# eigenkernel/eigenkernel

Hardware: AMD Instinct MI355X
Metric: eigenpairs/s (full spectrum) + achieved fp64 TFLOP/s vs roofline, N=16384 GEP (higher is better)
Workload: dtype f64

## Files before the change

### eigenkernel_amd/csrc/ek_api_internal.h

```cpp
#pragma once
#include "../../include/ek_hip.h"
#include "../../include/ek_hip_debug.h"
#include "ek_common.h"

#include <rccl/rccl.h>

#include <chrono>
#include <cstdlib>
#include <cstring>
#include <mutex>
#include <vector>

namespace ek {
namespace batched {
struct Desc {
  double *A, *B, *w, *Z;
  int n, lda, ldb, ldz, index, pad;
};
static_assert(sizeof(Desc) == 56, "the table's entry");
}

namespace api {

struct Context {
// ... 60 lines not shown
struct GridCell { int nb, nprow, npcol, myrow, mycol; };

extern ek_hip_allgatherv_fn g_allgatherv;
extern void *g_allgatherv_user;

int pad_ld(int n);
int h2d_matrix(int m, int n, const double *h, int ldh, double *d, int ldd, hipStream_t s);
int d2h_matrix(int m, int n, const double *d, int ldd, double *h, int ldh, hipStream_t s);
int fetch_info(int *info);
void poison_foreign_strips(hipStream_t s, int n, double *A, int lda, int P, int rank);
void count_mismatch(hipStream_t s, int m, int n, const double *X, int ldx, const double *Y, int ldy, int lower,
                    unsigned long long *count);

struct Comm {
  bool on = false;
  bool host = false;
  ncclComm_t comm = nullptr;
  int nranks = 0, rank = 0;
  int err = 0;
};
extern Comm g_comm;
constexpr int kPotrfRlMin = 1024;
extern int g_two_stage_min;
int two_stage_min();
int dist_min_ranks();
void comm_teardown();
SytrdExchange team_exchange(int nteam, int n = 0);
void team_sendrecv(hipStream_t s, int npeers, const int *peers, double *const *send, const size_t *send_counts,
                   double *const *recv, const size_t *recv_counts);
int comm_any(int local);
int comm_agree(int local_rc);
const char *comm_error_string();

void gather_band_strips(hipStream_t s, int n, int nmem, int rank0, double *const *ABs, const SytrdExchange &x);

}
}
```

### eigenkernel_amd/csrc/ek_comm.hip

```cpp
#include "ek_api_internal.h"
#include <dlfcn.h>

namespace ek {
namespace api {

struct Rccl {
  void *h = nullptr;
  ncclResult_t (*GetUniqueId)(ncclUniqueId *) = nullptr;
  ncclResult_t (*CommInitRank)(ncclComm_t *, int, ncclUniqueId, int) = nullptr;
  ncclResult_t (*CommDestroy)(ncclComm_t) = nullptr;
  ncclResult_t (*AllReduce)(const void *, void *, size_t, ncclDataType_t, ncclRedOp_t, ncclComm_t, hipStream_t) = nullptr;
  const char *(*GetErrorString)(ncclResult_t) = nullptr;
  ncclResult_t (*Broadcast)(const void *, void *, size_t, ncclDataType_t, int, ncclComm_t, hipStream_t) = nullptr;
  ncclResult_t (*GroupStart)() = nullptr;
  ncclResult_t (*GroupEnd)() = nullptr;
  ncclResult_t (*AllGather)(const void *, void *, size_t, ncclDataType_t, ncclComm_t, hipStream_t) = nullptr;
  ncclResult_t (*Send)(const void *, size_t, ncclDataType_t, int, ncclComm_t, hipStream_t) = nullptr;
  ncclResult_t (*Recv)(void *, size_t, ncclDataType_t, int, ncclComm_t, hipStream_t) = nullptr;
  int load() {
    if (h) return 0;
    const char *names[] = {getenv("EK_HIP_RCCL_LIB"), "librccl.so.1", "librccl.so", "/opt/rocm/lib/librccl.so.1"};
    for (const char *nm : names) {
      if (!nm || !*nm) continue;
      h = dlopen(nm, RTLD_NOW | RTLD_GLOBAL);
// ... 29 lines not shown
}

void rccl_allgatherv(hipStream_t s, int nmem, int, double *const *bufs, const size_t *offs,
                     const size_t *counts, int nranks, void *) {
  if (nmem != 1 || !g_comm.on || nranks != g_comm.nranks) { if (!g_comm.err) g_comm.err = (int)ncclInvalidUsage; return; }
  bool side_by_side = g_rccl.AllGather != nullptr && counts[0] > 0;
  for (int q = 1; q < nranks && side_by_side; ++q) side_by_side = counts[q] == counts[0] && offs[q] == offs[0] + (size_t)q * counts[0];
  if (side_by_side) {
    const ncclResult_t ra = g_rccl.AllGather(bufs[0] + offs[g_comm.rank], bufs[0] + offs[0], counts[0], ncclDouble, g_comm.comm, s);
    if (ra != ncclSuccess && !g_comm.err) g_comm.err = (int)ra;
    return;
  }
  ncclResult_t r = g_rccl.GroupStart();
  for (int root = 0; root < nranks && r == ncclSuccess; ++root)
    if (counts[root] > 0)
      r = g_rccl.Broadcast(bufs[0] + offs[root], bufs[0] + offs[root], counts[root], ncclDouble, root, g_comm.comm, s);
  const ncclResult_t r2 = g_rccl.GroupEnd();
  if (r == ncclSuccess) r = r2;
  if (r != ncclSuccess && !g_comm.err) g_comm.err = (int)r;
}


int g_two_stage_min = -1;
int two_stage_min() {
  if (g_two_stage_min >= 0) return g_two_stage_min;
  static int env = -2;
  if (env == -2) { const char *e = getenv("EK_HIP_TWO_STAGE_MIN"); env = e ? atoi(e) : -1; }
  return env >= 0 ? env : 512;
}

int dist_min_ranks() {
  const char *e = getenv("EK_HIP_DIST_MIN_RANKS");
  return e ? atoi(e) : 3;
}

std::vector<double> g_hx_send, g_hx_recv;
void host_allreduce(hipStream_t s, int nmem, double *const *bufs, size_t count, void *) {
  if (nmem != 1 || !g_comm.on || !g_allgatherv) { if (!g_comm.err) g_comm.err = (int)ncclInvalidUsage; return; }
  const int P = g_comm.nranks;
  g_hx_send.resize(count); g_hx_recv.resize(count * P);
  std::vector<long long> counts(P, (long long)count), displs(P);
  for (int r = 0; r < P; ++r) displs[r] = (long long)r * (long long)count;
  bool ok = hipStreamSynchronize(s) == hipSuccess &&
            hipMemcpy(g_hx_send.data(), bufs[0], count * 8, hipMemcpyDeviceToHost) == hipSuccess;
  if (ok) ok = g_allgatherv(g_hx_send.data(), (long long)count, g_hx_recv.data(), counts.data(), displs.data(),
                            g_allgatherv_user) == 0;
// ... 222 lines not shown
```

### eigenkernel_amd/csrc/ek_common.h

```cpp
#pragma once
#include <hip/hip_runtime.h>
#include <cstddef>
#include <cstdint>
#include <cstdio>

#define EK_HIP_CHECK(expr)                                                              \
  do {                                                                                  \
    hipError_t _e = (expr);                                                             \
    if (_e != hipSuccess) {                                                             \
      fprintf(stderr, "[ek_hip] %s failed at %s:%d: %s\n", #expr, __FILE__, __LINE__,   \
              hipGetErrorString(_e));                                                   \
      return -1000 - (int)_e;                                                           \
    }                                                                                   \
  } while (0)

namespace ek {

constexpr int kWave = 64;

inline int ceil_div(int a, int b) { return (a + b - 1) / b; }
inline int round_up(int a, int b) { return ceil_div(a, b) * b; }

struct GemmDesc {
  int M, N, K;
// ... 138 lines not shown
void symv_profile_collect(double *seconds, long long *launches, double *bytes);

constexpr int kBandW = 64;
size_t sy2sb_work_bytes(int n);
void sy2sb_lower(hipStream_t s, hipStream_t s2, int n, double *A, int lda, double *Vall, int ldv, double *tau1,
                 int *d_flag, void *work);

struct Sy2sbMember { double *A; int lda; double *Vall; int ldv; double *tau1; int *d_flag; void *work; int rank; };
size_t sy2sb_dist_work_bytes(int n, int nranks);
void sy2sb_lower_dist(hipStream_t s, hipStream_t s2, int n, int nmem, const Sy2sbMember *mem, const SytrdExchange &x);
void sy2sb_dist_set_lookahead(int min_rows);
void sy2sb_dist_profile(bool on);
void sy2sb_dist_profile_collect(double *seconds, int P);

size_t sb2st_work_bytes(int n, bool with_records = true);
size_t sb2st_record_bytes(int n);
constexpr int kBandLd = 2 * kBandW;
double *sb2st_band(void *work, int n);
void pack_band(hipStream_t s, int n, const double *A, int lda, double *AB );
void sb2st_lower(hipStream_t s, int n, const double *A, int lda, double *d, double *e, double *V2, int ldv2,
                 int *d_flag, void *work, bool band_packed = false, int chase_mode = 0);
void sb2st_apply_q2(hipStream_t s, int n, int ncols, const double *V2, int ldv2, double *Z, int ldz, int *d_flag,
                    void *work, double *records = nullptr);

size_t stedc_work_bytes(int n, int nsel = -1);
bool stedc_compact(int n, int nsel);
struct StedcSelect { int nsel, nb, npcol, mycol; int first = 0; };
struct StedcTeam { int nranks; int rank; const SytrdExchange *x; int levels; };
int stedc_team_levels(int n, int nranks);
void stedc_team_set_levels(int levels);
void stedc_team_profile(bool on);
void stedc_team_profile_collect(double *seconds);
void stedc(hipStream_t s, int n, const double *d, const double *e, double *w, double *Z,
           int ldz, void *work, int *d_info, const StedcSelect *sel = nullptr, double *d_flops = nullptr,
           double *wscratch = nullptr, const StedcTeam *team = nullptr);

size_t stebz_work_bytes(int n);
void stebz(hipStream_t s, int n, const double *d, const double *e, int il, int iu, double *w, void *work);
int stebz_set_lanes(int lanes);
int *stebz_window(hipStream_t s, int n, const double *d, const double *e, double vl, double vu, void *work);

size_t ormtr_work_bytes(int n, int ncols, int ncols_global = -1);
void ormtr_lower(hipStream_t s, int n, int ncols, const double *V, int ldv, const double *tau,
                 double *Z, int ldz, void *work, int ncols_global = -1);
size_t ormtr_prep_bytes(int n);
void ormtr_prepare(hipStream_t s, int n, const double *V, int ldv, const double *tau, void *prep);
// ... 18 lines not shown
```

### eigenkernel_amd/csrc/ek_debug.hip

```cpp
#include "ek_api_internal.h"

using namespace ek;
using namespace ek::api;

extern "C" {

int ek_hip_potrf_team(int n, double *B_loc, const int desc_B[9], int nteam, long long *mismatch) {
  if (n < 0) return -1;
  if (!B_loc && n > 0) return -2;
  int rc = check_desc(desc_B, 3, n, n); if (rc) return rc;
  if (nteam < 0 || nteam > kMaxTeam) return -4;
  rc = ensure_init(); if (rc) return rc;
  if (mismatch) *mismatch = 0;
  if (n == 0) return 0;
  std::lock_guard<std::mutex> lk(g_mu);
  if (nteam == 0 && !g_comm.on) return -4;
  hipStream_t s = g_ctx.stream;
  const int ld = pad_ld(n), nblk = ceil_div(n, kDiagNB);
  const int nmem = nteam > 0 ? nteam : 1, P = nteam > 0 ? nteam : g_comm.nranks;
  const size_t wb = potrf_dist_work_bytes(n, ld, P);
  const size_t per = al((size_t)ld * ld * 8) + al((size_t)nblk * kDiagNB * kDiagNB * 8) + al(wb) + 256;
  void *ws;
  rc = workspace(per * nmem + 256, &ws);
  if (rc) return rc;
// ... 289 lines not shown
  double *dd = a.get<double>(ld), *de = a.get<double>(ld);
  EK_HIP_CHECK(hipMemsetAsync(dA, 0, (size_t)ld * ld * 8, s));
  EK_HIP_CHECK(hipMemsetAsync(dV2, 0, (size_t)ld * ld * 8, s));
  EK_HIP_CHECK(hipMemsetAsync(dd, 0, 2 * al((size_t)ld * 8), s));
  EK_HIP_CHECK(hipMemsetAsync(g_ctx.d_info, 0, 4 * sizeof(int), s));
  rc = h2d_matrix(n, n, A, lda, dA, ld, s); if (rc) return rc;
  sb2st_lower(s, n, dA, ld, dd, de, dV2, ld, g_ctx.d_info + 2, work);
  if (ncols > 0) {
    rc = h2d_matrix(n, ncols, Z, ldz, dZ, ld, s); if (rc) return rc;
    sb2st_apply_q2(s, n, ncols, dV2, ld, dZ, ld, g_ctx.d_info + 2, work);
    rc = d2h_matrix(n, ncols, dZ, ld, Z, ldz, s); if (rc) return rc;
  }
  EK_HIP_CHECK(hipGetLastError());
  EK_HIP_CHECK(hipMemcpyAsync(d, dd, (size_t)n * 8, hipMemcpyDeviceToHost, s));
  if (n > 1) EK_HIP_CHECK(hipMemcpyAsync(e, de, (size_t)(n - 1) * 8, hipMemcpyDeviceToHost, s));
  int f = 0;
  EK_HIP_CHECK(hipMemcpyAsync(&f, g_ctx.d_info + 2, sizeof(int), hipMemcpyDeviceToHost, s));
  EK_HIP_CHECK(hipStreamSynchronize(s));
  if (flag) *flag = f;
  return 0;
}

int ek_hip_debug_set_two_stage(int min_order) { g_two_stage_min = min_order; return 0; }

int ek_hip_profile_kernels(int enable) {
  int rc = ensure_init(); if (rc) return rc;
  std::lock_guard<std::mutex> lk(g_mu);
  EK_HIP_CHECK(hipStreamSynchronize(g_ctx.stream));
  kprof_enable(enable != 0);
  return 0;
}
int ek_hip_profile_kernels_get(double *seconds, long long *launches) {
  int rc = ensure_init(); if (rc) return rc;
  std::lock_guard<std::mutex> lk(g_mu);
  EK_HIP_CHECK(hipStreamSynchronize(g_ctx.stream));
  kprof_collect(seconds, launches);
  return 0;
}

int ek_hip_debug_last_solve_stats(double *out, int count) {
  std::lock_guard<std::mutex> lk(g_mu);
  for (int i = 0; i < count && i < 8; ++i) out[i] = g_ctx.stats[i];
  return 0;
}

int ek_hip_debug_two_stage_timing(int n, int ncols, int reps, double *seconds, int *flag) {
// ... 407 lines not shown
```

### eigenkernel_amd/csrc/ek_sb2st.hip

```cpp
#include "ek_common.h"

#include <cstdlib>
#include <type_traits>
#include <vector>

namespace ek {
namespace {

typedef double double4_t __attribute__((ext_vector_type(4)));

constexpr int SB = kBandW;
constexpr int LDAB = 2 * SB;
constexpr int DLD = SB + 1;

__device__ __forceinline__ double ld_sc1(const double *p) {
  return __longlong_as_double((long long)__hip_atomic_load((const unsigned long long *)p, __ATOMIC_RELAXED,
                                                           __HIP_MEMORY_SCOPE_AGENT));
}
__device__ __forceinline__ void st_sc1(double *p, double v) {
  __hip_atomic_store((unsigned long long *)p, (unsigned long long)__double_as_longlong(v), __ATOMIC_RELAXED,
                     __HIP_MEMORY_SCOPE_AGENT);
}
template <int CTRL>
__device__ __forceinline__ double dpp_mov(double v) {
// ... 1095 lines not shown
    if (nw == 16) hipLaunchKernelGGL(chase_kernel<16>, dim3(nwg), dim3(1024), 0, s, c);
    else if (nw == 8) hipLaunchKernelGGL(chase_kernel<8>, dim3(nwg), dim3(512), 0, s, c);
    else hipLaunchKernelGGL(chase_kernel<4>, dim3(nwg), dim3(256), 0, s, c);
    kprof_end(s, kProfChase);
  }
  hipLaunchKernelGGL(unpack_de_kernel, dim3(ceil_div(n, 256)), dim3(256), 0, s, n, AB, d, e);
  if (getenv("EK_SB2ST_PROF")) {
    long long h[8];
    (void)hipMemcpyAsync(h, ctl + 16, sizeof(h), hipMemcpyDeviceToHost, s);
    (void)hipStreamSynchronize(s);
    fprintf(stderr, "[sb2st prof] tasks %lld; cycles per task: gate+loads %.0f, reflector %.0f, left-apply+fill %.0f, "
            "partials %.0f, updates %.0f\n", h[6], (double)h[0] / h[6], (double)h[1] / h[6], (double)h[2] / h[6],
            (double)h[3] / h[6], (double)h[4] / h[6]);
  }
  if (getenv("EK_SB2ST_VERBOSE")) {
    unsigned h[8];
    (void)hipMemcpyAsync(h, ctl, sizeof(h), hipMemcpyDeviceToHost, s);
    (void)hipStreamSynchronize(s);
    fprintf(stderr, "[sb2st] n %d: abort %u, positions abandoned %u, census %u\n", n, h[1], h[3], h[4]);
  }
  hipLaunchKernelGGL(forward_abort_kernel, dim3(1), dim3(1), 0, s, ctl, d_flag);
}

void sb2st_apply_q2(hipStream_t s, int n, int ncols, const double *V2, int ldv2, double *Z, int ldz, int *d_flag,
                    void *work, double *records) {
  if (n <= 2 || ncols <= 0) return;
  const Layout L(n, records == nullptr);
  char *w = (char *)work;
  const double *tau2 = (const double *)(w + L.off_tau);
  double *Rec = records ? records : (double *)(w + L.off_T);
  unsigned *ctl = (unsigned *)(w + L.off_ctl), *qprog = (unsigned *)(w + L.off_qprog);
  unsigned *offS = (unsigned *)(w + L.off_offs);
  hipLaunchKernelGGL(q2_offsets_kernel, dim3(1), dim3(64), 0, s, n, L.nS, offS);
  Q2Geom g{n, L.nsweeps, L.nS, L.kmax, offS};
  hipLaunchKernelGGL(q2_tfactor_kernel, dim3(L.kmax, L.nS), dim3(256), 0, s, g, V2, ldv2, tau2, L.ldt, Rec);
  constexpr size_t lds = (size_t)(QOPSZ + 4 * 16 * QSTLD) * sizeof(double);
  static bool attr = false;
  if (!attr) {
    (void)hipFuncSetAttribute((const void *)q2_apply_nb_kernel<2>, hipFuncAttributeMaxDynamicSharedMemorySize, (int)lds);
    (void)hipFuncSetAttribute((const void *)q2_apply_nb_kernel<3>, hipFuncAttributeMaxDynamicSharedMemorySize, (int)lds);
    (void)hipFuncSetAttribute((const void *)q2_apply_nb_kernel<4>, hipFuncAttributeMaxDynamicSharedMemorySize, (int)lds);
    attr = true;
  }
  int nblk = (n >= 8192) ? 4 : 3;
  if (const char *ev = getenv("EK_Q2_NBLK")) { const int v = atoi(ev); if (v >= 2 && v <= 4) nblk = v; }
  const int per = nblk;
  const int nslab = ceil_div(ncols, QNC), npair = ceil_div(L.nS, per), npass = npair * nslab;
  (void)hipMemsetAsync(qprog, 0, (size_t)npass * 4, s);
  (void)hipMemsetAsync(ctl + 2, 0, 4, s);
  Q2ApplyArgs a{g, Rec, Z, ldz, ncols, nslab, npass, npair, qprog, ctl, 0};
  if (const char *ev = getenv("EK_Q2_EXTRA")) a.extra = atoi(ev);
  int nwg = 512;
  if (const char *ev = getenv("EK_Q2_WGS")) { const int v = atoi(ev); if (v > 0) nwg = v; }
  if (nwg > npass) nwg = npass;
  kprof_begin(s, kProfQ2Apply);
  if (nblk == 3) hipLaunchKernelGGL(q2_apply_nb_kernel<3>, dim3(nwg), dim3(256), lds, s, a);
  else if (nblk == 4) hipLaunchKernelGGL(q2_apply_nb_kernel<4>, dim3(nwg), dim3(256), lds, s, a);
  else hipLaunchKernelGGL(q2_apply_nb_kernel<2>, dim3(nwg), dim3(256), lds, s, a);
  kprof_end(s, kProfQ2Apply);
  if (d_flag) hipLaunchKernelGGL(forward_abort_kernel, dim3(1), dim3(1), 0, s, ctl, d_flag);
}

}
```

### eigenkernel_amd/csrc/ek_solve.hip

```cpp
#include "ek_api_internal.h"

#include <condition_variable>
#include <sched.h>
#include <deque>
#include <memory>
#include <new>
#include <thread>

namespace ek {
namespace api {

void gather_band_strips(hipStream_t s, int n, int nmem, int rank0, double *const *ABs, const SytrdExchange &x) {
  const int NRB = ceil_div(n, 128), P = x.nranks;
  if (P <= 1) return;
  for (int q = 0; q * P < NRB; ++q) {
    size_t offs[kMaxTeam], counts[kMaxTeam];
    for (int r = 0; r < P; ++r) {
      const int S = q * P + r;
      const int cols = (S < NRB) ? ((n - S * 128 < 128) ? n - S * 128 : 128) : 0;
      offs[r] = (S < NRB) ? (size_t)S * 128 * kBandLd : 0; counts[r] = (size_t)cols * kBandLd;
    }
    x.allgatherv(s, nmem, rank0, ABs, offs, counts, P, x.user);
  }
}
// ... 391 lines not shown
    return alias_env && p && n % 128 == 0 && ldu == ld && (((size_t)p) & 255) == 0;
  };
  const bool aliasA = alias_ok(dA, lda), aliasB = problem == 1 && alias_ok(dB, ldb);
  const bool aliasZ = !values_only && !value_window && !cell && nc_loc == n && zcols == ld && alias_ok(dZ, ldz);
  double *wB = aliasB ? dB : a.get<double>((size_t)ld * ld);
  double *wV = a.get<double>((size_t)ld * ld);
  double *wZ = (aliasZ || values_only) ? dZ : a.get<double>((size_t)ld * zcols);
  double *x0 = a.get<double>((size_t)ld * ld);
  char *x1 = a.get<char>(pl.x1);
  double *dInv = a.get<double>((size_t)nblk * kDiagNB * kDiagNB);
  double *twork = a.get<double>((size_t)256 * ld);
  double *dd = a.get<double>(ld), *de = a.get<double>(ld), *dt = a.get<double>(ld), *dwv = a.get<double>(ld);
  double *dt1 = a.get<double>(ld);
  char *work_sy2sb = two_stage ? a.get<char>(pl.wb_sy2sb) : nullptr;
  char *work_sb2st = two_stage ? a.get<char>(pl.wb_sb2st) : nullptr;
  char *q1prep = (two_stage && !values_only) ? a.get<char>(pl.wb_q1prep) : nullptr;
  double *inv256 = pl.inv256 ? (double *)a.get<char>(pl.inv256) : nullptr;
  struct Inv256Guard { ~Inv256Guard() { trsm_register_inv256(nullptr, nullptr, 0); } } inv256_guard;
  double *wA = aliasA ? dA : x0;
  double *wV2 = x0;
  double *sscr = (problem == 1) ? (double *)x1 : nullptr;
  char *pwork = pl.potrf_wb ? x1 + al(pl.sygst_dbl * 8) : nullptr;
  char *work = x1;
  double *q2rec = (double *)x1;
  char *sytrd_arena = x1 + al(pl.sygst_dbl * 8) + pl.potrf_wb + 256;
  void *sytrd_work = two_stage ? nullptr : choose_sytrd_scratch(n, ld, x0, sytrd_arena, dd, wb_sytrd);

  StageTimer tm;
  const bool timing = stage_seconds && n_stages > 0;
  if (timing) { rc = tm.init(); if (rc) return rc; }
  int evi = 0;
  auto mark = [&]() { if (timing) (void)hipEventRecord(tm.ev[evi++], s); };

  EK_HIP_CHECK(hipMemsetAsync(g_ctx.d_info, 0, 4 * sizeof(int), s));
  mark();
  EK_HIP_CHECK(hipMemsetAsync(wV, 0, (size_t)ld * ld * 8, s));
  EK_HIP_CHECK(hipMemsetAsync(dd, 0, 4 * al((size_t)ld * 8), s));
  double sigma = 1.0;
  bool band_input = false;
  auto stage_in_B = [&]() -> int {
    if (problem != 1) return 0;
    if (pipe) { const int e = pipe->wait_in(0); if (e) return e; }
    if (aliasB) return 0;
    if (ld != n) EK_HIP_CHECK(hipMemsetAsync(wB, 0, (size_t)ld * ld * 8, s));
    copy_matrix(s, n, n, dB, ldb, wB, ld);
    return 0;
  };
// ... 114 lines not shown
      EK_HIP_CHECK(hipStreamSynchronize(s));
      win->il = ilu[0]; win->iu = ilu[1] >= ilu[0] ? ilu[1] : ilu[0] - 1;
    }
    win->first = win->il - 1;
    win->m = win->iu - win->il + 1;
    window_too_small = win->jobz == 1 && win->m > win->zcap;
  }
  if (values_only || (win && (win->m == 0 || window_too_small))) {
    const int m = win->m;
    if (values_only && m > 0) stebz(s, n, dd, de, win->il, win->iu, dwv, x1);
    mark(); mark(); mark();
    if (values_only && m > 0 && sigma != 1.0) scale_vector(s, m, 1.0 / sigma, dwv);
    if (values_only && m > 0) EK_HIP_CHECK(hipMemcpyAsync(dw, dwv, (size_t)m * 8, hipMemcpyDeviceToDevice, s));
    if (problem == 1 && !aliasB) copy_matrix(s, n, n, wB, ld, dB, ldb);
    mark();
    EK_HIP_CHECK(hipGetLastError());
    int info[4] = {0, 0, 0, 0};
    EK_HIP_CHECK(hipMemcpyAsync(info, g_ctx.d_info, sizeof(info), hipMemcpyDeviceToHost, s));
    EK_HIP_CHECK(hipStreamSynchronize(s));
    g_ctx.stats[0] = 0.0;
    g_ctx.stats[1] = two_stage_done ? 1.0 : 0.0;
    g_ctx.stats[2] = rescued_panels;
    g_ctx.stats[3] = (two_stage_done && band_input) ? 1.0 : 0.0;
    if (timing) {
      float ms[8];
      for (int i = 0; i < 8; ++i) (void)hipEventElapsedTime(&ms[i], tm.ev[i], tm.ev[i + 1]);
      double st[EK_HIP_N_STAGES] = {0};
      st[EK_STAGE_COPY] = (ms[0] + ms[7]) * 1e-3;
      st[EK_STAGE_POTRF] = ms[1] * 1e-3; st[EK_STAGE_SYGST] = ms[2] * 1e-3;
      st[EK_STAGE_SYTRD] = ms[3] * 1e-3; st[EK_STAGE_STEDC] = ms[4] * 1e-3;
      for (int i = 0; i < n_stages && i < EK_HIP_N_STAGES; ++i) stage_seconds[i] = st[i];
      tm.destroy();
    }
    if (info[0] != 0) return info[0];
    return window_too_small ? kWindowTooSmall : 0;
  }
  if (value_window) { nc_loc = win->m; n_vec = win->m; }
  const StedcSelect pick{nc_loc, cell ? cell->nb : (n > 0 ? n : 1), split_rows ? g_comm.nranks : (cell ? cell->npcol : 1),
                         split_rows ? g_comm.rank : (cell ? cell->mycol : 0), win ? win->first : 0};
  SytrdExchange dcx{};
  StedcTeam dct{0, 0, nullptr, 0};
  if (dist && g_comm.nranks >= 2) {
    const int P = g_comm.nranks, nbz = cell->nb, Pc = split_rows ? P : cell->npcol;
    bool all_compact = true;
    for (int r = 0; r < Pc; ++r) all_compact = all_compact && stedc_compact(n, numroc0(n_vec, nbz, r, Pc));
    dcx = team_exchange(0);
    dct = StedcTeam{P, g_comm.rank, &dcx, all_compact ? stedc_team_levels(n, P) : 0};
  }
  else if (cell && !dist && g_debug_dc_team >= 2) dct = StedcTeam{g_debug_dc_team, -1, nullptr, stedc_team_levels(n, g_debug_dc_team)};
  stedc(s, n, dd, de, dwv, wZ, ld, work, g_ctx.d_info + 1, &pick, g_ctx.d_stats, nullptr, dct.levels > 0 ? &dct : nullptr);
  mark();
  double *zc = wZ;
  const int zslab = (pipe && two_stage_done && nc_loc > pipe->z_slab) ? pipe->z_slab : nc_loc;
  auto slab_width = [&](int c0) {
    const int left = nc_loc - c0;
    if (zslab >= nc_loc) return left;
    if (left > 2 * zslab) return zslab;
    if (left > zslab) return zslab / 2 < left ? zslab / 2 : left;
    return (left > 512) ? (left + 1) / 2 : left;
  };
  auto z_out = [&](int c0, int nc) {
    if (!aliasZ) copy_matrix(s, n, nc, wZ + (size_t)c0 * ld, ld, dZ + (size_t)c0 * ldz, ldz);
    pipe->push(true, dZ + (size_t)c0 * ldz, ldz, pipe->hZ + (size_t)c0 * pipe->ldhz, pipe->ldhz, n, nc, pipe->mark(s), 0);
  };
  if (two_stage_done) {
    sb2st_apply_q2(s, n, nc_loc, wV2, ld, zc, ld, g_ctx.d_info + 2, work_sb2st, q2rec);
    const bool q1 = !band_input;
    if (q1) ormtr_prepare(s, n, wV, ld, dt1, q1prep);
    if (pipe && problem == 0 && zslab < nc_loc) {
      for (int c0 = 0, nc = 0; c0 < nc_loc; c0 += nc) {
        nc = slab_width(c0);
        if (q1) ormtr_apply(s, n, nc, wV, ld, q1prep, zc + (size_t)c0 * ld, ld, work, n_vec);
        z_out(c0, nc);
      }
    } else if (q1) {
      ormtr_apply(s, n, nc_loc, wV, ld, q1prep, zc, ld, work, n_vec);
    }
  } else {
    ormtr_lower(s, n, nc_loc, wV, ld, dt, zc, ld, work, n_vec);
  }
  mark();
  if (problem == 1) {
    if (itype == 3) trmm_diag_blocks(s, n, wB, ld, wV);
    auto recover = [&](int nc, double *zp) {
      if (itype == 3) trmm_lln(s, n, nc, wB, ld, wV, trmm_block_ld(n), zp, ld, twork);
      else trsm_llt(s, n, nc, wB, ld, dInv, zp, ld, twork);
    };
    if (pipe) {
      for (int c0 = 0, nc = 0; c0 < nc_loc; c0 += nc) {
        nc = slab_width(c0);
        recover(nc, zc + (size_t)c0 * ld);
// ... 30 lines not shown
        rcn[q] = (size_t)nr_loc * numroc0(n_vec, nb, i * C + cell->mycol, P);
        rp[q] = buf; buf += rcn[q]; ++q;
      }
      team_sendrecv(s, np, peers, sp, sc, rp, rcn);
      const int ldp = nr_loc > 1 ? nr_loc : 1;
      for (int i = 0, q = 0; i < R; ++i) {
        const int nc_i = numroc0(n_vec, nb, i * C + cell->mycol, P);
        const double *src = (i == cell->myrow) ? own : rp[q++];
        scatter_block_cyclic(s, nr_loc, nc_i, src, ldp, nb, 1, 0, R, i, dZ, ldz);
      }
    } else if (cell) gather_block_cyclic(s, nr_loc, nc_loc, zc, ld, cell->nb, cell->nprow, cell->myrow, 1, 0, dZ, ldz);
    else if (!aliasZ) copy_matrix(s, n, n_vec, wZ, ld, dZ, ldz);
    if (problem == 1 && !aliasB) copy_matrix(s, n, n, wB, ld, dB, ldb);
  }
  mark();
  EK_HIP_CHECK(hipGetLastError());
  int info[4] = {0, 0, 0, 0};
  EK_HIP_CHECK(hipMemcpyAsync(info, g_ctx.d_info, sizeof(info), hipMemcpyDeviceToHost, s));
  EK_HIP_CHECK(hipMemcpyAsync(g_ctx.stats, g_ctx.d_stats, sizeof(g_ctx.stats), hipMemcpyDeviceToHost, s));
  EK_HIP_CHECK(hipStreamSynchronize(s));
  g_ctx.stats[1] = two_stage_done ? 1.0 : 0.0;
  g_ctx.stats[2] = rescued_panels;
  g_ctx.stats[3] = (two_stage_done && band_input) ? 1.0 : 0.0;
  info[2] &= 0xff;
  if (timing) {
    float ms[8];
    for (int i = 0; i < 8; ++i) (void)hipEventElapsedTime(&ms[i], tm.ev[i], tm.ev[i + 1]);
    double st[EK_HIP_N_STAGES] = {0};
    st[EK_STAGE_COPY] = (ms[0] + ms[7]) * 1e-3;
    st[EK_STAGE_POTRF] = ms[1] * 1e-3; st[EK_STAGE_SYGST] = ms[2] * 1e-3;
    st[EK_STAGE_SYTRD] = ms[3] * 1e-3; st[EK_STAGE_GATHER] = 0.0;
    st[EK_STAGE_STEDC] = ms[4] * 1e-3; st[EK_STAGE_ORMTR] = ms[5] * 1e-3;
    st[EK_STAGE_TRTRS] = ms[6] * 1e-3;
    for (int i = 0; i < n_stages && i < EK_HIP_N_STAGES; ++i) stage_seconds[i] = st[i];
    tm.destroy();
  }
  int bad = two_stage_done && info[2] != 0;
  if (dist) {
    bad = comm_any(bad);
    if (bad < 0) {
      if (g_comm.err) fprintf(stderr, "[ek_hip] exchange failed: %s\n", comm_error_string());
      return -996;
    }
  }
  if (bad) return -992;
  if (info[0] != 0) return info[0];
// ... 611 lines not shown
```

### eigenkernel_amd/solver.py

```python
import ctypes
import os
from dataclasses import dataclass, field

import numpy as np

from . import descriptor as _d

_HERE = os.path.dirname(os.path.abspath(__file__))
LIB_PATH = os.environ.get("EK_HIP_LIB") or os.path.join(_HERE, "csrc", "libek_hip.so")

N_STAGES = 8
SOLVERS = ("hip", "hip_select", "general_hip", "general_hip_select")
REPLACES = {"hip": "scalapack", "hip_select": "scalapack_select",
            "general_hip": "general_scalapack", "general_hip_select": "general_scalapack_select"}


class LibraryMissing(RuntimeError):
    pass


_lib = None
_dp = ctypes.POINTER(ctypes.c_double)
_ip = ctypes.POINTER(ctypes.c_int)
_llp = ctypes.POINTER(ctypes.c_longlong)
# ... 64 lines not shown
        "ek_hip_debug_sytrd_work_bytes": (ctypes.c_ulonglong, [c_int]),
        "ek_hip_debug_sytrd_split": (c_int, [vp, c_int]),
        "ek_hip_debug_gemm_at": (c_int, [c_int, c_int, c_int, c_int, c_int, vp, c_int, vp, c_int, c_dbl, vp, c_int,
                                         c_int, c_int, _dp]),
        "ek_hip_debug_sytrd_at": (c_int, [c_int, c_int, c_int, vp, vp, vp, _dp]),
        "ek_hip_debug_gemm_desc": (c_int, [c_int] * 5 + [c_dbl, c_dbl, vp, c_int, c_ll, vp, c_int, c_ll, vp, c_int, c_ll]
                                   + [c_int] * 5 + [_llp, _ip, _ip]),
        "ek_hip_debug_gemm_plan": (c_int, [c_int] * 5 + [c_dbl, c_dbl, vp, c_int, c_ll, vp, c_int, c_ll, vp, c_int, c_ll]
                                   + [c_int] * 5 + [_llp, _ip, _ip]),
        "ek_hip_debug_gemm_compact_map": (c_int, [c_int, c_int, c_ll, c_int, _ip, _ip, _ip]),
        "ek_hip_debug_reduce_team": (c_int, [c_int, c_int, c_int, _dp]),
        "ek_hip_profile_symv_get": (c_int, [_dp, ctypes.POINTER(ctypes.c_longlong), _dp]),
        "ek_hip_debug_sy2sb": (c_int, [c_int, _dp, c_int, _dp, c_int, _dp, _ip]),
        "ek_hip_debug_sb2st": (c_int, [c_int, _dp, c_int, _dp, _dp, _dp, c_int, c_int, _ip]),
        "ek_hip_debug_two_stage_timing": (c_int, [c_int, c_int, c_int, _dp, _ip]),
        "ek_hip_debug_set_two_stage": (c_int, [c_int]),
        "ek_hip_profile_kernels": (c_int, [c_int]),
        "ek_hip_profile_kernels_get": (c_int, [_dp, _llp]),
        "ek_hip_debug_last_solve_stats": (c_int, [_dp, c_int]),
        "ek_hip_debug_sy2sb_team": (c_int, [c_int, _dp, c_int, _dp, c_int, _dp, c_int, _ip, _llp]),
        "ek_hip_debug_sy2sb_team_timing": (c_int, [c_int, c_int, c_int, _dp]),
        "ek_hip_debug_sy2sb_team_profile": (c_int, [c_int, c_int, c_int, c_int, _dp, _dp]),
        "ek_hip_debug_fail_next_chase": (c_int, [c_int]),
        "ek_hip_debug_stedc_team": (c_int, [c_int, c_int, c_int]),
        "ek_hip_debug_potrf_team_profile": (c_int, [c_int, c_int]),
        "ek_hip_debug_potrf_team_profile_get": (c_int, [c_int, _dp]),
        "ek_hip_debug_stedc_team_get": (c_int, [_dp]),
        "ek_hip_debug_last_pipe_stats": (c_int, [_dp, c_int]),
        "ek_hip_debug_workspace_bytes": (ctypes.c_ulonglong, [c_int, c_int, c_int, c_int, ctypes.POINTER(ctypes.c_ulonglong)]),
        "ek_hip_eigenvalues_device": (c_int, [c_int, c_int, c_int, c_int, vp, c_int, vp, c_int, vp, _dp, c_int]),
        "ek_hip_eigenvalues": (c_int, [c_int, c_int, c_int, c_int, _dp, c_int, _dp, c_int, _dp, _dp, c_int]),
        "ek_hip_stebz": (c_int, [c_int, _dp, _dp, c_int, c_int, _dp]),
        "ek_hip_debug_values_workspace_bytes": (ctypes.c_ulonglong, [c_int, c_int]),
        "ek_hip_debug_set_stebz": (c_int, [c_int]),
        "ek_hip_eigenpairs_device": (c_int, [c_int, c_int, c_int, c_int, c_dbl, c_dbl, c_int, c_int, vp, c_int, vp, c_int,
                                             _ip, _ip, vp, vp, c_int, c_int, _dp, c_int]),
        "ek_hip_eigenpairs": (c_int, [c_int, c_int, c_int, c_int, c_dbl, c_dbl, c_int, c_int, _dp, c_int, _dp, c_int,
                                      _ip, _ip, _dp, _dp, c_int, c_int, _dp, c_int]),
        "ek_hip_stebz_range": (c_int, [c_int, _dp, _dp, c_dbl, c_dbl, _ip, _ip, _dp]),
        "ek_hip_debug_window_workspace_bytes": (ctypes.c_ulonglong, [c_int, c_int, c_int, c_int, c_int]),
        "ek_hip_sygvx_device": (c_int, [c_int, c_int, c_int, c_int, c_dbl, c_dbl, c_int, c_int, vp, c_int, vp, c_int,
                                        _ip, _ip, vp, vp, c_int, c_int, _dp, c_int]),
        "ek_hip_sygvx": (c_int, [c_int, c_int, c_int, c_int, c_dbl, c_dbl, c_int, c_int, _dp, c_int, _dp, c_int,
                                 _ip, _ip, _dp, _dp, c_int, c_int, _dp, c_int]),
        "ek_hip_sygst_ibtype": (c_int, [c_int, c_int, _dp, _ip, _dp, _ip, _dp]),
        "ek_hip_trmm": (c_int, [c_int, c_int, _dp, _ip, _dp, _ip]),
# ... 62 lines not shown
            raise
        fn.restype = res
        fn.argtypes = args
    if path is None:
        _lib = lib
    return lib


EXPORTED_SYMBOLS = (
    "ek_hip_version", "ek_hip_init", "ek_hip_finalize", "ek_hip_stage_name", "ek_hip_solve",
    "ek_hip_solve_device", "ek_hip_solve_replicated", "ek_hip_solve_device_grid",
    "ek_hip_set_allgatherv", "ek_hip_gather_matrix", "ek_hip_potrf", "ek_hip_sygst", "ek_hip_sytrd", "ek_hip_stedc",
    "ek_hip_ormtr", "ek_hip_trtrs", "ek_hip_dgemm", "ek_hip_malloc", "ek_hip_free",
    "ek_hip_memcpy_h2d", "ek_hip_memcpy_d2h", "ek_hip_synchronize", "ek_hip_synth_matrix_device",
    "ek_hip_profile_symv", "ek_hip_profile_symv_get", "ek_hip_debug_sytrd",
    "ek_hip_residual_device", "ek_hip_orthogonality_device", "ek_hip_ipratios_device", "ek_hip_check",
    "ek_hip_sytrd_team", "ek_hip_comm_unique_id", "ek_hip_comm_init", "ek_hip_comm_size", "ek_hip_comm_rank",
    "ek_hip_comm_destroy", "ek_hip_comm_allreduce_device", "ek_hip_debug_sytrd_team", "ek_hip_sygst_team",
    "ek_hip_potrf_team", "ek_hip_debug_reduce_team", "ek_hip_comm_attach_host",
    "ek_hip_debug_set_sytrd_maxcols", "ek_hip_debug_sytrd_work_bytes", "ek_hip_debug_sytrd_at", "ek_hip_debug_sytrd_split", "ek_hip_debug_gemm_at",
    "ek_hip_debug_gemm_desc", "ek_hip_debug_gemm_plan", "ek_hip_debug_gemm_compact_map",
    "ek_hip_debug_sy2sb", "ek_hip_debug_sb2st", "ek_hip_debug_two_stage_timing", "ek_hip_debug_set_two_stage",
    "ek_hip_profile_kernels", "ek_hip_profile_kernels_get", "ek_hip_debug_last_solve_stats",
    "ek_hip_debug_sy2sb_team", "ek_hip_debug_sy2sb_team_timing", "ek_hip_debug_sy2sb_team_profile", "ek_hip_debug_workspace_bytes", "ek_hip_debug_fail_next_chase", "ek_hip_debug_last_pipe_stats",
    "ek_hip_debug_stedc_team", "ek_hip_debug_stedc_team_get",
    "ek_hip_debug_potrf_team_profile", "ek_hip_debug_potrf_team_profile_get",
    "ek_hip_eigenvalues_device", "ek_hip_eigenvalues", "ek_hip_stebz",
    "ek_hip_debug_values_workspace_bytes", "ek_hip_debug_set_stebz",
    "ek_hip_eigenpairs_device", "ek_hip_eigenpairs", "ek_hip_stebz_range", "ek_hip_debug_window_workspace_bytes",
    "ek_hip_sygvx_device", "ek_hip_sygvx", "ek_hip_sygst_ibtype", "ek_hip_trmm", "ek_hip_debug_sygvx_workspace_bytes",
    "ek_hip_eigenpairs_batched_device", "ek_hip_eigenpairs_batched",
    "ek_hip_eigenpairs_vbatched_device", "ek_hip_eigenpairs_vbatched",
    "ek_hip_debug_vbatched_streams", "ek_hip_debug_vbatched_last",
    "ek_hip_check_batched_device", "ek_hip_check_batched", "ek_hip_check_vbatched_device", "ek_hip_check_vbatched",
    "ek_hip_sygv_batched_device", "ek_hip_sygv_batched", "ek_hip_sygv_vbatched_device", "ek_hip_sygv_vbatched",
    "ek_hip_check_sygv_batched_device", "ek_hip_check_sygv_batched", "ek_hip_check_sygv_vbatched_device",
    "ek_hip_check_sygv_vbatched", "ek_hip_check_sygvx_device", "ek_hip_check_sygvx",
    "ek_hip_eigenpairs_xbatched_device", "ek_hip_eigenpairs_xbatched", "ek_hip_debug_xbatched_chunk",
    "ek_hip_check_xbatched_device", "ek_hip_check_xbatched", "ek_hip_debug_check_xbatched_chunk",
    "ek_hip_sygv_xbatched_device", "ek_hip_sygv_xbatched",
    "ek_hip_check_sygv_xbatched_device", "ek_hip_check_sygv_xbatched",
    "ek_hip_eigenpairs_xvbatched_device", "ek_hip_eigenpairs_xvbatched", "ek_hip_sygv_xvbatched_device",
    "ek_hip_sygv_xvbatched", "ek_hip_debug_xvbatched_last",
)


def _check(what, A, B, w, Z, n_cols, index1=1, index2=1):
# ... 284 lines not shown
def sygst_ibtype(A, L, ibtype):
    lib = load_library()
    A = np.array(_farr(A), order="F", copy=True)
    L = _farr(L)
    scale = ctypes.c_double(0.0)
    info = lib.ek_hip_sygst_ibtype(int(ibtype), A.shape[0], _P(A), _I(_desc_for(A)), _P(L), _I(_desc_for(L)),
                                   ctypes.byref(scale))
    return A, info


def trmm(L, Z):
    lib = load_library()
    L = _farr(L)
    Z = np.array(_farr(Z), order="F", copy=True)
    info = lib.ek_hip_trmm(L.shape[0], Z.shape[1], _P(L), _I(_desc_for(L)), _P(Z), _I(_desc_for(Z)))
    return Z, info


BAND_W = 64


def set_two_stage(min_order=-1):
    load_library().ek_hip_debug_set_two_stage(int(min_order))


def stedc_team(nranks=0, levels=-1, profile=False):
    rc = load_library().ek_hip_debug_stedc_team(int(nranks), int(levels), 1 if profile else 0)
    assert rc == 0, rc


def stedc_team_seconds():
    out = (ctypes.c_double * 3)()
    rc = load_library().ek_hip_debug_stedc_team_get(out)
    assert rc == 0, rc
    return [float(x) for x in out]


def last_solve_stats():
    st = (ctypes.c_double * 8)()
    load_library().ek_hip_debug_last_solve_stats(st, 8)
    return [float(x) for x in st]


def workspace_bytes(problem, n, n_vec=None, nranks=1):
    parts = (ctypes.c_ulonglong * 6)()
    tot = load_library().ek_hip_debug_workspace_bytes(int(problem), int(n), int(n if n_vec is None else n_vec), int(nranks), parts)
# ... 501 lines not shown
```

### include/ek_hip_debug.h

```cpp
#ifndef EK_HIP_DEBUG_H
#define EK_HIP_DEBUG_H

#ifdef __cplusplus
extern "C" {
#endif

int ek_hip_profile_symv(int enable);
int ek_hip_profile_symv_get(double *seconds, long long *launches, double *algorithmic_bytes);

int ek_hip_profile_kernels(int enable);
int ek_hip_profile_kernels_get(double *seconds , long long *launches );

int ek_hip_debug_sytrd(int n, int ld, int reps, double *seconds);
unsigned long long ek_hip_debug_sytrd_work_bytes(int n);
int ek_hip_debug_sytrd_at(int n, int max_cols, int reps, double *dA, void *work, double *vecs, double *seconds);
int ek_hip_debug_gemm_at(int transa, int transb, int m, int n, int k, const double *dA, int lda, const double *dB,
                         int ldb, double beta, double *dC, int ldc, int lower_only, int reps, double *seconds);
int ek_hip_debug_gemm_desc(int transa, int transb, int m, int n, int k, double alpha, double beta, const double *dA, int lda,
                           long long strideA, const double *dB, int ldb, long long strideB, double *dC, int ldc,
                           long long strideC, int batch, int lower_only, int staged_rank_k, int small_tiles, int even_offs,
                           const long long *offs, const int *dims, int *variant );
int ek_hip_debug_gemm_plan(int transa, int transb, int m, int n, int k, double alpha, double beta, const double *dA, int lda,
                           long long strideA, const double *dB, int ldb, long long strideB, double *dC, int ldc,
                           long long strideC, int batch, int lower_only, int staged_rank_k, int small_tiles, int even_offs,
// ... 7 lines not shown
int ek_hip_debug_sy2sb(int n, double *A, int lda, double *V, int ldv, double *tau, int *flag);
int ek_hip_debug_sb2st(int n, const double *A, int lda, double *d, double *e, double *Z, int ldz, int ncols, int *flag);
int ek_hip_debug_two_stage_timing(int n, int ncols, int reps, double *seconds, int *flag);
int ek_hip_debug_set_two_stage(int min_order);
int ek_hip_debug_sy2sb_team(int n, double *A, int lda, double *V, int ldv, double *tau, int nteam, int *flag,
                            long long *mismatch);
int ek_hip_debug_sy2sb_team_timing(int n, int nteam, int reps, double *seconds);
int ek_hip_debug_sy2sb_team_profile(int n, int nteam, int reps, int lookahead_min, double *seconds, double *parts);

int ek_hip_debug_last_solve_stats(double *out, int count);

unsigned long long ek_hip_debug_workspace_bytes(int problem, int n, int n_vec, int nranks, unsigned long long *parts);

unsigned long long ek_hip_debug_values_workspace_bytes(int problem, int n);
int ek_hip_debug_set_stebz(int lanes);
unsigned long long ek_hip_debug_window_workspace_bytes(int problem, int n, int jobz, int range, int m);
unsigned long long ek_hip_debug_sygvx_workspace_bytes(int itype, int n, int jobz, int range, int m);
int ek_hip_debug_vbatched_streams(int streams);
int ek_hip_debug_vbatched_last(double *class_seconds, int *class_count);
int ek_hip_debug_xvbatched_last(double *class_seconds, int *class_count);
int ek_hip_debug_xbatched_chunk(int problems);
int ek_hip_debug_check_xbatched_chunk(int problems);

int ek_hip_debug_fail_next_chase(int times);

int ek_hip_debug_stedc_team(int nranks, int levels, int profile);
int ek_hip_debug_stedc_team_get(double *seconds);

int ek_hip_debug_potrf_team_profile(int lookahead, int profile);
int ek_hip_debug_potrf_team_profile_get(int nteam, double *parts);

int ek_hip_debug_last_pipe_stats(double *out, int count);

#ifdef __cplusplus
}
#endif
#endif
```

Baseline: 19620.

## Overlap Q2 T-factor and Q1 ormtr preparation with stedc on a second stream

Splits the sb2st Q2 back-transform into a prepare phase (offsets plus T-factor kernels) and an apply phase. When two-stage reduction ran and a second stream exists, the Q2 and Q1 preparation is forked onto stream2 so it runs concurrently with the tridiagonal divide-and-conquer (stedc), then joined before the apply. To avoid clobbering the shared scratch that stedc uses, the Q2 records get their own arena slice only when aliased matrix space is large enough. This adds event sync and extra concurrent GPU load during stedc, and workspace aliasing could be a correctness risk.

Result: no change. 19710, median of 6 (+0.5%).

```diff
diff --git a/eigenkernel_amd/csrc/ek_api_internal.h b/eigenkernel_amd/csrc/ek_api_internal.h
--- a/eigenkernel_amd/csrc/ek_api_internal.h
+++ b/eigenkernel_amd/csrc/ek_api_internal.h
@@ -106,6 +106,7 @@
 extern Comm g_comm;
 constexpr int kPotrfRlMin = 1024;
 extern int g_two_stage_min;
+extern int g_prep_overlap;
 int two_stage_min();
 int dist_min_ranks();
 void comm_teardown();
diff --git a/eigenkernel_amd/csrc/ek_comm.hip b/eigenkernel_amd/csrc/ek_comm.hip
--- a/eigenkernel_amd/csrc/ek_comm.hip
+++ b/eigenkernel_amd/csrc/ek_comm.hip
@@ -75,6 +75,7 @@
 
 
 int g_two_stage_min = -1;
+int g_prep_overlap = 1;
 int two_stage_min() {
   if (g_two_stage_min >= 0) return g_two_stage_min;
   static int env = -2;
diff --git a/eigenkernel_amd/csrc/ek_common.h b/eigenkernel_amd/csrc/ek_common.h
--- a/eigenkernel_amd/csrc/ek_common.h
+++ b/eigenkernel_amd/csrc/ek_common.h
@@ -184,6 +184,9 @@
                  int *d_flag, void *work, bool band_packed = false, int chase_mode = 0);
 void sb2st_apply_q2(hipStream_t s, int n, int ncols, const double *V2, int ldv2, double *Z, int ldz, int *d_flag,
                     void *work, double *records = nullptr);
+void sb2st_prepare_q2(hipStream_t s, int n, const double *V2, int ldv2, void *work, double *records = nullptr);
+void sb2st_apply_q2_prepared(hipStream_t s, int n, int ncols, double *Z, int ldz, int *d_flag, void *work,
+                             double *records = nullptr);
 
 size_t stedc_work_bytes(int n, int nsel = -1);
 bool stedc_compact(int n, int nsel);
diff --git a/eigenkernel_amd/csrc/ek_debug.hip b/eigenkernel_amd/csrc/ek_debug.hip
--- a/eigenkernel_amd/csrc/ek_debug.hip
+++ b/eigenkernel_amd/csrc/ek_debug.hip
@@ -335,6 +335,12 @@
 }
 
 int ek_hip_debug_set_two_stage(int min_order) { g_two_stage_min = min_order; return 0; }
+int ek_hip_debug_set_prep_overlap(int on) {
+  std::lock_guard<std::mutex> lk(g_mu);
+  const int was = g_prep_overlap;
+  g_prep_overlap = on != 0 ? 1 : 0;
+  return was;
+}
 
 int ek_hip_profile_kernels(int enable) {
   int rc = ensure_init(); if (rc) return rc;
diff --git a/eigenkernel_amd/csrc/ek_sb2st.hip b/eigenkernel_amd/csrc/ek_sb2st.hip
--- a/eigenkernel_amd/csrc/ek_sb2st.hip
+++ b/eigenkernel_amd/csrc/ek_sb2st.hip
@@ -1141,18 +1141,27 @@
   hipLaunchKernelGGL(forward_abort_kernel, dim3(1), dim3(1), 0, s, ctl, d_flag);
 }
 
-void sb2st_apply_q2(hipStream_t s, int n, int ncols, const double *V2, int ldv2, double *Z, int ldz, int *d_flag,
-                    void *work, double *records) {
-  if (n <= 2 || ncols <= 0) return;
+void sb2st_prepare_q2(hipStream_t s, int n, const double *V2, int ldv2, void *work, double *records) {
+  if (n <= 2) return;
   const Layout L(n, records == nullptr);
   char *w = (char *)work;
   const double *tau2 = (const double *)(w + L.off_tau);
   double *Rec = records ? records : (double *)(w + L.off_T);
-  unsigned *ctl = (unsigned *)(w + L.off_ctl), *qprog = (unsigned *)(w + L.off_qprog);
   unsigned *offS = (unsigned *)(w + L.off_offs);
   hipLaunchKernelGGL(q2_offsets_kernel, dim3(1), dim3(64), 0, s, n, L.nS, offS);
   Q2Geom g{n, L.nsweeps, L.nS, L.kmax, offS};
   hipLaunchKernelGGL(q2_tfactor_kernel, dim3(L.kmax, L.nS), dim3(256), 0, s, g, V2, ldv2, tau2, L.ldt, Rec);
+}
+
+void sb2st_apply_q2_prepared(hipStream_t s, int n, int ncols, double *Z, int ldz, int *d_flag, void *work,
+                             double *records) {
+  if (n <= 2 || ncols <= 0) return;
+  const Layout L(n, records == nullptr);
+  char *w = (char *)work;
+  double *Rec = records ? records : (double *)(w + L.off_T);
+  unsigned *ctl = (unsigned *)(w + L.off_ctl), *qprog = (unsigned *)(w + L.off_qprog);
+  unsigned *offS = (unsigned *)(w + L.off_offs);
+  Q2Geom g{n, L.nsweeps, L.nS, L.kmax, offS};
   constexpr size_t lds = (size_t)(QOPSZ + 4 * 16 * QSTLD) * sizeof(double);
   static bool attr = false;
   if (!attr) {
@@ -1180,4 +1189,11 @@
   if (d_flag) hipLaunchKernelGGL(forward_abort_kernel, dim3(1), dim3(1), 0, s, ctl, d_flag);
 }
 
-}
+void sb2st_apply_q2(hipStream_t s, int n, int ncols, const double *V2, int ldv2, double *Z, int ldz, int *d_flag,
+                    void *work, double *records) {
+  if (n <= 2 || ncols <= 0) return;
+  sb2st_prepare_q2(s, n, V2, ldv2, work, records);
+  sb2st_apply_q2_prepared(s, n, ncols, Z, ldz, d_flag, work, records);
+}
+
+}
diff --git a/eigenkernel_amd/csrc/ek_solve.hip b/eigenkernel_amd/csrc/ek_solve.hip
--- a/eigenkernel_amd/csrc/ek_solve.hip
+++ b/eigenkernel_amd/csrc/ek_solve.hip
@@ -437,7 +437,9 @@
   double *sscr = (problem == 1) ? (double *)x1 : nullptr;
   char *pwork = pl.potrf_wb ? x1 + al(pl.sygst_dbl * 8) : nullptr;
   char *work = x1;
-  double *q2rec = (double *)x1;
+  const bool rec_own = two_stage && !values_only && pl.wb_rec > 0 &&
+                       (aliasB ? pl.mat : 0) + (aliasZ ? pl.zmat : 0) >= pl.wb_rec;
+  double *q2rec = rec_own ? (double *)a.get<char>(pl.wb_rec) : (double *)x1;
   char *sytrd_arena = x1 + al(pl.sygst_dbl * 8) + pl.potrf_wb + 256;
   void *sytrd_work = two_stage ? nullptr : choose_sytrd_scratch(n, ld, x0, sytrd_arena, dd, wb_sytrd);
 
@@ -598,6 +600,7 @@
     g_ctx.stats[1] = two_stage_done ? 1.0 : 0.0;
     g_ctx.stats[2] = rescued_panels;
     g_ctx.stats[3] = (two_stage_done && band_input) ? 1.0 : 0.0;
+    g_ctx.stats[4] = 0.0;
     if (timing) {
       float ms[8];
       for (int i = 0; i < 8; ++i) (void)hipEventElapsedTime(&ms[i], tm.ev[i], tm.ev[i + 1]);
@@ -624,6 +627,29 @@
     dct = StedcTeam{P, g_comm.rank, &dcx, all_compact ? stedc_team_levels(n, P) : 0};
   }
   else if (cell && !dist && g_debug_dc_team >= 2) dct = StedcTeam{g_debug_dc_team, -1, nullptr, stedc_team_levels(n, g_debug_dc_team)};
+  const bool q1 = two_stage_done && !band_input;
+  const bool fork = two_stage_done && g_prep_overlap != 0 && g_ctx.stream2 && (rec_own || q1);
+  struct PrepJoin {
+    hipStream_t s; hipEvent_t ev; bool pending;
+    void join() { if (pending) { (void)hipStreamWaitEvent(s, ev, 0); pending = false; } }
+    ~PrepJoin() { join(); }
+  } prep{s, nullptr, false};
+  if (fork) {
+    static bool evs = false;
+    static hipEvent_t ev_fork, ev_join;
+    if (!evs) {
+      EK_HIP_CHECK(hipEventCreateWithFlags(&ev_fork, hipEventDisableTiming));
+      EK_HIP_CHECK(hipEventCreateWithFlags(&ev_join, hipEventDisableTiming));
+      evs = true;
+    }
+    hipStream_t s2 = g_ctx.stream2;
+    EK_HIP_CHECK(hipEventRecord(ev_fork, s));
+    EK_HIP_CHECK(hipStreamWaitEvent(s2, ev_fork, 0));
+    if (rec_own) sb2st_prepare_q2(s2, n, wV2, ld, work_sb2st, q2rec);
+    if (q1) ormtr_prepare(s2, n, wV, ld, dt1, q1prep);
+    EK_HIP_CHECK(hipEventRecord(ev_join, s2));
+    prep.ev = ev_join; prep.pending = true;
+  }
   stedc(s, n, dd, de, dwv, wZ, ld, work, g_ctx.d_info + 1, &pick, g_ctx.d_stats, nullptr, dct.levels > 0 ? &dct : nullptr);
   mark();
   double *zc = wZ;
@@ -640,9 +666,10 @@
     pipe->push(true, dZ + (size_t)c0 * ldz, ldz, pipe->hZ + (size_t)c0 * pipe->ldhz, pipe->ldhz, n, nc, pipe->mark(s), 0);
   };
   if (two_stage_done) {
-    sb2st_apply_q2(s, n, nc_loc, wV2, ld, zc, ld, g_ctx.d_info + 2, work_sb2st, q2rec);
-    const bool q1 = !band_input;
-    if (q1) ormtr_prepare(s, n, wV, ld, dt1, q1prep);
+    if (!(fork && rec_own)) sb2st_prepare_q2(s, n, wV2, ld, work_sb2st, q2rec);
+    prep.join();
+    sb2st_apply_q2_prepared(s, n, nc_loc, zc, ld, g_ctx.d_info + 2, work_sb2st, q2rec);
+    if (q1 && !fork) ormtr_prepare(s, n, wV, ld, dt1, q1prep);
     if (pipe && problem == 0 && zslab < nc_loc) {
       for (int c0 = 0, nc = 0; c0 < nc_loc; c0 += nc) {
         nc = slab_width(c0);
@@ -719,6 +746,7 @@
   g_ctx.stats[1] = two_stage_done ? 1.0 : 0.0;
   g_ctx.stats[2] = rescued_panels;
   g_ctx.stats[3] = (two_stage_done && band_input) ? 1.0 : 0.0;
+  g_ctx.stats[4] = fork ? (q1 ? 1.0 : 0.0) + (rec_own ? 2.0 : 0.0) : 0.0;
   info[2] &= 0xff;
   if (timing) {
     float ms[8];
diff --git a/eigenkernel_amd/solver.py b/eigenkernel_amd/solver.py
--- a/eigenkernel_amd/solver.py
+++ b/eigenkernel_amd/solver.py
@@ -110,6 +110,7 @@
         "ek_hip_debug_sy2sb_team_timing": (c_int, [c_int, c_int, c_int, _dp]),
         "ek_hip_debug_sy2sb_team_profile": (c_int, [c_int, c_int, c_int, c_int, _dp, _dp]),
         "ek_hip_debug_fail_next_chase": (c_int, [c_int]),
+        "ek_hip_debug_set_prep_overlap": (c_int, [c_int]),
         "ek_hip_debug_stedc_team": (c_int, [c_int, c_int, c_int]),
         "ek_hip_debug_potrf_team_profile": (c_int, [c_int, c_int]),
         "ek_hip_debug_potrf_team_profile_get": (c_int, [c_int, _dp]),
@@ -218,7 +219,7 @@
     "ek_hip_debug_gemm_desc", "ek_hip_debug_gemm_plan", "ek_hip_debug_gemm_compact_map",
     "ek_hip_debug_sy2sb", "ek_hip_debug_sb2st", "ek_hip_debug_two_stage_timing", "ek_hip_debug_set_two_stage",
     "ek_hip_profile_kernels", "ek_hip_profile_kernels_get", "ek_hip_debug_last_solve_stats",
-    "ek_hip_debug_sy2sb_team", "ek_hip_debug_sy2sb_team_timing", "ek_hip_debug_sy2sb_team_profile", "ek_hip_debug_workspace_bytes", "ek_hip_debug_fail_next_chase", "ek_hip_debug_last_pipe_stats",
+    "ek_hip_debug_sy2sb_team", "ek_hip_debug_sy2sb_team_timing", "ek_hip_debug_sy2sb_team_profile", "ek_hip_debug_workspace_bytes", "ek_hip_debug_fail_next_chase", "ek_hip_debug_set_prep_overlap", "ek_hip_debug_last_pipe_stats",
     "ek_hip_debug_stedc_team", "ek_hip_debug_stedc_team_get",
     "ek_hip_debug_potrf_team_profile", "ek_hip_debug_potrf_team_profile_get",
     "ek_hip_eigenvalues_device", "ek_hip_eigenvalues", "ek_hip_stebz",
@@ -549,6 +550,10 @@
 
 def set_two_stage(min_order=-1):
     load_library().ek_hip_debug_set_two_stage(int(min_order))
+
+
+def set_prep_overlap(on=True):
+    return bool(load_library().ek_hip_debug_set_prep_overlap(1 if on else 0))
 
 
 def stedc_team(nranks=0, levels=-1, profile=False):
diff --git a/include/ek_hip_debug.h b/include/ek_hip_debug.h
--- a/include/ek_hip_debug.h
+++ b/include/ek_hip_debug.h
@@ -53,6 +53,8 @@
 int ek_hip_debug_xbatched_chunk(int problems);
 int ek_hip_debug_check_xbatched_chunk(int problems);
 
+int ek_hip_debug_set_prep_overlap(int on);
+
 int ek_hip_debug_fail_next_chase(int times);
 
 int ek_hip_debug_stedc_team(int nranks, int levels, int profile);
```
